# linkedin/spark-tfrecord

Hardware: NVIDIA H100
Metric: TFRecord decode GB/s (1 KB Example, 64 mixed features) at 1/2/4/8 H100 (higher is better)
Workload: dtype u8

## Files before the change

### spark-tfrecord_b200/_native.py

```python
from __future__ import annotations

import ctypes as C
import os
from typing import List, Optional

import numpy as np

from . import _cabi as A
from ._cabi import HostColumn, column_from_ctypes, make_fields, tfr_batch_info, tfr_column, tfr_field
from .sqltypes import StructType

_DIR = os.path.dirname(os.path.abspath(__file__))
LIB_PATH = os.environ.get("TFR_LIB") or os.path.join(_DIR, "libtfrgpu.so")
_LIB = None

EXPORTS = [
    "tfr_abi_version", "tfr_status_string", "tfr_last_error", "tfr_schema_create", "tfr_schema_destroy",
    "tfr_schema_num_fields", "tfr_decoder_create", "tfr_decoder_destroy", "tfr_decoder_staging", "tfr_decoder_staging_slot",
    "tfr_decoder_num_staging_slots", "tfr_decode", "tfr_decode_submit",
    "tfr_decoder_stream", "tfr_decoder_set_profiling", "tfr_decoder_get_profile", "tfr_decoder_get_stats", "tfr_batch_wait", "tfr_batch_status", "tfr_batch_consumed", "tfr_batch_num_columns", "tfr_batch_columns",
    "tfr_batch_to_host_async", "tfr_batch_to_host", "tfr_batch_export_arrow_host", "tfr_batch_export_arrow_device", "tfr_batch_release",
    "tfr_encoder_create", "tfr_encoder_destroy", "tfr_encode", "tfr_encoder_result_host", "tfr_encoder_stream",
    "tfr_infer_create", "tfr_infer_update", "tfr_infer_update_block", "tfr_infer_result", "tfr_infer_name", "tfr_infer_destroy",
]
# ... 232 lines not shown
        h = C.c_void_p()
        _check(lib().tfr_decoder_create(self.schema.h, device, flags, C.byref(h)))
        self.h = h

    def staging(self, nbytes: int) -> np.ndarray:
        p = C.c_void_p()
        cap = C.c_size_t()
        _check(lib().tfr_decoder_staging(self.h, nbytes, C.byref(p), C.byref(cap)))
        return np.ctypeslib.as_array(C.cast(p, C.POINTER(C.c_uint8)), shape=(cap.value,))

    def staging_slot(self, slot: int, nbytes: int) -> np.ndarray:
        p = C.c_void_p()
        cap = C.c_size_t()
        _check(lib().tfr_decoder_staging_slot(self.h, slot, nbytes, C.byref(p), C.byref(cap)))
        return np.ctypeslib.as_array(C.cast(p, C.POINTER(C.c_uint8)), shape=(cap.value,))

    @staticmethod
    def num_staging_slots() -> int:
        return lib().tfr_decoder_num_staging_slots()

    def stats(self) -> dict:
        v = (C.c_int64 * 8)()
        _check(lib().tfr_decoder_get_stats(self.h, v, 8))
        names = ["batches", "speculative_submits", "speculative_redone", "count_mode_batches", "general_path_batches", "shapes_learned", "transcode_reruns"]
        return {k: v[i] for i, k in enumerate(names)}

    def stream(self) -> int:
        p = C.c_void_p()
        _check(lib().tfr_decoder_stream(self.h, C.byref(p)))
        return p.value or 0

    def set_profiling(self, enable: bool):
        _check(lib().tfr_decoder_set_profiling(self.h, 1 if enable else 0))

    def get_profile(self):
        ms = (C.c_double * 8)()
        nl = C.c_int64()
        n1 = C.c_int64()
        _check(lib().tfr_decoder_get_profile(self.h, ms, C.byref(nl), C.byref(n1)))
        names = ["frame_index", "pass1", "scan", "pass2", "pack_validity", "h2d", "d2h"]
        return {"ms": {k: ms[i] for i, k in enumerate(names)}, "launches": nl.value, "pass1_launches": n1.value}

    def decode(self, data, is_final: bool = True, nbytes: Optional[int] = None):
        ptr, n, on_dev, keep = _device_ptr(data)
        if nbytes is not None:
            n = nbytes
        b = C.c_void_p()
# ... 113 lines not shown
```

### spark-tfrecord_b200/csrc/api_decode.inc

```

static inline size_t align_up(size_t v, size_t a) { return (v + a - 1) / a * a; }

struct HostStats {
  FrameResult frame;
  DecodeSummary summary;
  uint32_t overflow;
  uint32_t pad[3];
};

struct K1Bufs {
  DevBuf chunks, chunk_base, first, stage, rec_off;
  uint32_t n_chunks = 0, chunk_bytes = 0;
  void release() { chunks.release(); chunk_base.release(); first.release(); stage.release(); rec_off.release(); }
};

struct PtrTables {
  void** h = nullptr; size_t cap = 0;
  DevBuf dev;
  int32_t ensure(size_t n_ptr) {
    if (cap < n_ptr) {
      if (h) cudaFreeHost(h);
      h = nullptr; cap = 0;
      CUDA_TRY(cudaHostAlloc((void**)&h, n_ptr * sizeof(void*), cudaHostAllocDefault));
      cap = n_ptr;
// ... 50 lines not shown
  Lane lanes[TFR_LANES];
  int next_lane = 0;
  HostStats* h_stats = nullptr;
  int64_t* h_totals = nullptr;
  PinnedPool host_pool;
  DevPool dev_pool;
  std::vector<cudaEvent_t> done_pool;
  bool fast_ok = false;
  int spec_state = 0;
  int relearn_backoff = 0;
  int shape_misses = 0;
  double mean_rec_bytes = 0.0;
  uint32_t last_max_len = 0;
  uint32_t last_max_tile = 0;
  int xc_batches = 0;
  double cap_slack = 0.0625;
  std::vector<int32_t> spec_len;
  bool spec_ragged = false;
  std::vector<double> hist_ratio;
  DevBuf uniform_dev;
  DevBuf no_uniform_dev;
  int32_t* h_uniform = nullptr;
  int64_t stats[8] = {0};
  bool profiling = false;
  struct Span { int stage; cudaEvent_t a, b; };
  std::vector<Span> spans;
  std::vector<cudaEvent_t> ev_pool;
  double prof_ms[TFR_PROFILE_STAGES] = {0};
  int64_t launches = 0, pass1_launches = 0;
  cudaEvent_t ev_get() {
    if (!ev_pool.empty()) { cudaEvent_t e = ev_pool.back(); ev_pool.pop_back(); return e; }
    cudaEvent_t e; cudaEventCreate(&e); return e;
  }
  void span_begin(int stage, cudaStream_t st = nullptr) { if (!profiling) return; Span s{stage, ev_get(), nullptr}; cudaEventRecord(s.a, st ? st : stream); spans.push_back(s); }
  void span_end(int nlaunch, cudaStream_t st = nullptr) { launches += nlaunch; if (!profiling) return; Span& s = spans.back(); s.b = ev_get(); cudaEventRecord(s.b, st ? st : stream); }
  void spans_resolve() {
    const bool trace = !spans.empty() && getenv("TFR_TRACE");
    for (auto& s : spans) {
      if (!s.b) { ev_pool.push_back(s.a); continue; }
      float ms = 0; if (cudaEventElapsedTime(&ms, s.a, s.b) == cudaSuccess) prof_ms[s.stage] += ms;
      if (trace) { float t0 = 0; cudaEventElapsedTime(&t0, spans[0].a, s.a); fprintf(stderr, "tfr_trace stage %d start %.3f end %.3f\n", s.stage, t0, t0 + ms); }
      ev_pool.push_back(s.a); ev_pool.push_back(s.b);
    }
    spans.clear();
  }
};

struct tfr_batch {
  tfr_decoder* dec = nullptr;
  std::atomic<int> refs{1};
  tfr_batch_info info{};
  std::vector<tfr_column> cols;
  std::vector<tfr_column> host_cols;
  void* dev_fixed = nullptr; size_t dev_fixed_bytes = 0;
  void* dev_var = nullptr; size_t dev_var_bytes = 0;
  unsigned long long* d_null_counts = nullptr;
  std::vector<unsigned long long> h_null_counts_tmp;
  void* host_copy = nullptr; size_t host_copy_bytes = 0;
  bool host_copy_enqueued = false;
  cudaEvent_t d2h_done = nullptr;
  bool null_counts_ready = false;
  cudaEvent_t done = nullptr;
  bool pending = false;
  Lane* lane = nullptr;
  const void* src = nullptr; size_t src_bytes = 0; int src_on_device = 0, is_final = 0;
  bool xc_tried = false;
  OutLayout lay;
  std::vector<size_t> lvl_off;
  std::vector<int32_t> uni_len;
};

static void give_event(tfr_decoder* d, cudaEvent_t e) { if (e) d->done_pool.push_back(e); }
static int32_t take_event(tfr_decoder* d, cudaEvent_t* e) {
  if (!d->done_pool.empty()) { *e = d->done_pool.back(); d->done_pool.pop_back(); return TFR_OK; }
  CUDA_TRY(cudaEventCreateWithFlags(e, cudaEventDisableTiming));
  return TFR_OK;
}

extern "C" int32_t tfr_decoder_create(const tfr_schema* schema, int32_t device, uint32_t flags, tfr_decoder** out) {
  if (!schema || !out) return fail(TFR_E_INVALID_ARG, "null argument");
  DeviceCtx* ctx = nullptr;
  int32_t rc = get_ctx(device, &ctx);
  if (rc) return rc;
  CUDA_TRY(cudaSetDevice(device));
  auto* d = new tfr_decoder;
  d->schema = *schema; d->device = device; d->flags = flags; d->ctx = ctx;
  CUDA_TRY(cudaStreamCreateWithFlags(&d->stream, cudaStreamNonBlocking));
  {
    int lo = 0, hi = 0;
    CUDA_TRY(cudaDeviceGetStreamPriorityRange(&lo, &hi));
    CUDA_TRY(cudaStreamCreateWithPriority(&d->st_k1, cudaStreamNonBlocking, getenv("TFR_NO_K1_PRIORITY") ? lo : hi));
  }
  CUDA_TRY(cudaStreamCreateWithFlags(&d->st_h2d, cudaStreamNonBlocking));
  CUDA_TRY(cudaStreamCreateWithFlags(&d->st_d2h, cudaStreamNonBlocking));
  CUDA_TRY(cudaStreamCreateWithFlags(&d->st_aux, cudaStreamNonBlocking));
  rc = d->dsch.upload(d->schema);
  if (!rc) rc = d->dsch.build_tile_consts(d->schema, ctx->d_tabs);
  if (rc) { delete d; return rc; }
  TRY(d->small.ensure(4096 + (size_t)d->schema.n_cnt * 16));
  {
    bool ok = d->schema.fields.size() <= 128 && !getenv("TFR_DISABLE_FAST");
    for (const DevField& f : d->schema.fields) if (f.depth > 1 && d->schema.record_type == TFR_RT_EXAMPLE) ok = false;
    d->fast_ok = ok;
    if (getenv("TFR_DISABLE_SPECULATION")) d->spec_state = -1;
    const size_t nv = std::max(1, d->schema.n_var);
    d->spec_len.assign(nv, -1);
    d->hist_ratio.assign(std::max(1, d->schema.n_cnt), 0.0);
    CUDA_TRY(cudaHostAlloc((void**)&d->h_uniform, nv * 4, cudaHostAllocDefault));
    TRY(d->uniform_dev.ensure(nv * 4));
    TRY(d->no_uniform_dev.ensure(nv * 4));
    CUDA_TRY(cudaMemset(d->no_uniform_dev.p, 0xff, nv * 4));
  }
  CUDA_TRY(cudaHostAlloc((void**)&d->h_stats, sizeof(HostStats), cudaHostAllocDefault));
  size_t nt = (size_t)d->schema.n_cnt * 2 + d->schema.fields.size() + 8;
  CUDA_TRY(cudaHostAlloc((void**)&d->h_totals, nt * sizeof(int64_t), cudaHostAllocDefault));
  for (Lane& L : d->lanes) {
    L.h_res_bytes = sizeof(LaneResult) + 8 * std::max<size_t>(1, d->schema.fields.size()) + 8 * std::max<size_t>(1, (size_t)d->schema.n_cnt);
    TRY(L.res.ensure(L.h_res_bytes));
    CUDA_TRY(cudaHostAlloc((void**)&L.h_res, L.h_res_bytes, cudaHostAllocDefault));
    CUDA_TRY(cudaEventCreateWithFlags(&L.ev_in, cudaEventDisableTiming));
    CUDA_TRY(cudaEventCreateWithFlags(&L.ev_k1, cudaEventDisableTiming));
    CUDA_TRY(cudaEventCreateWithFlags(&L.ev_tile, cudaEventDisableTiming));
    CUDA_TRY(cudaEventCreateWithFlags(&L.ev_frame, cudaEventDisableTiming));
    CUDA_TRY(cudaHostAlloc((void**)&L.h_frame, sizeof(FrameResult), cudaHostAllocDefault));
  }
  *out = d;
  return TFR_OK;
}
static void decoder_unref(tfr_decoder* d);
extern "C" void tfr_decoder_destroy(tfr_decoder* d) { if (d) decoder_unref(d); }
static void decoder_unref(tfr_decoder* d) {
  if (d->refs.fetch_sub(1) != 1) return;
  int prev = -1; cudaGetDevice(&prev);
  cudaSetDevice(d->device);
  for (cudaStream_t s : {d->st_h2d, d->st_k1, d->stream, d->st_d2h, d->st_aux}) cudaStreamSynchronize(s);
  for (DevBuf* b : {&d->in, &d->status, &d->valid8, &d->cnt, &d->src, &d->cflag, &d->tsum, &d->scan_scratch, &d->small, &d->uniform_dev, &d->no_uniform_dev})
    b->release();
  d->k1.release(); d->pt.release();
  for (Lane& L : d->lanes) {
    L.in.release(); L.k1.release(); L.res.release(); L.pt.release(); L.lb.release();
    if (L.h_res) cudaFreeHost(L.h_res);
    if (L.staging) cudaFreeHost(L.staging);
    if (L.ev_in) cudaEventDestroy(L.ev_in);
    if (L.ev_k1) cudaEventDestroy(L.ev_k1);
    if (L.ev_tile) cudaEventDestroy(L.ev_tile);
    if (L.ev_frame) cudaEventDestroy(L.ev_frame);
    if (L.h_frame) cudaFreeHost(L.h_frame);
    if (L.orphan_done) cudaEventDestroy(L.orphan_done);
  }
  d->dsch.free_all();
  cudaFreeHost(d->h_stats); cudaFreeHost(d->h_totals);
  if (d->h_uniform) cudaFreeHost(d->h_uniform);
  d->host_pool.release_all();
  d->dev_pool.release_all();
  for (cudaEvent_t e : d->done_pool) cudaEventDestroy(e);
  d->spans_resolve();
  for (cudaEvent_t e : d->ev_pool) cudaEventDestroy(e);
  for (cudaStream_t s : {d->st_h2d, d->st_k1, d->stream, d->st_d2h, d->st_aux}) cudaStreamDestroy(s);
  delete d;
// ... 303 lines not shown
        A.canon_lean = 1;
        const unsigned long long wgroups = (unsigned long long)((n_eff + 31) / 32) * S.n_var;
        const uint32_t gl = (uint32_t)std::min<unsigned long long>((wgroups + 7) / 8, (unsigned long long)d->ctx->sm_count * 48);
        decode_pass2_canon_kernel<<<std::max<uint32_t>(gl, 1), 256, 0, st>>>(A);
        ++nl2;
      }
      decode_pass2_kernel<<<g2, warps * 32, 0, st>>>(A);
      d->span_end(nl2);
    }
  }
  if (pack && n_eff > 0 && nf > 0) {
    uint32_t nbytes_bm = (n_eff + 7) / 8;
    dim3 g((nbytes_bm + 255) / 256, nf);
    g.x = std::min<uint32_t>(g.x, 4096);
    d->span_begin(4);
    pack_validity_kernel<<<g, 256, 0, st>>>((const uint8_t*)d->valid8.p, n, n_eff, nf, L.nb_stride, C.fx + L.bitmaps_off, b->d_null_counts);
    d->span_end(1);
  }
  build_views(b, S, n_eff, totals, lvl_off);
  return TFR_OK;
}

struct TileGeom { uint32_t tile_cap; uint32_t slot; bool small; size_t smem; uint32_t pf_dist; };
static TileGeom tile_geom_for(const tfr_decoder* d, uint32_t max_len, bool fill, uint32_t rg = 0, uint32_t max_tile = 0) {
  const uint32_t nf = (uint32_t)d->schema.fields.size(), nb = (uint32_t)d->schema.names.size();
  static const size_t l1_keep = getenv("TFR_L1_KEEP_KB") ? (size_t)atoi(getenv("TFR_L1_KEEP_KB")) << 10 : (size_t)16 << 10;
  const size_t sm_bytes = d->ctx->smem_per_sm;
  size_t stride = align_up((size_t)max_len + 16 + 15 + 32, 16);
  if (((stride >> 4) & 1) == 0) stride += 16;
  stride = std::min<size_t>(stride, 1u << 20);
  const size_t cap_fixed = stride * TILE_ROWS;
  TileGeom g;
  auto tiles_per_sm = [&](size_t cap, bool small) { return std::min<size_t>(sm_bytes / (tile_smem_bytes(nf, nb, (uint32_t)cap, rg) + 1024), small ? 8 : TILE_MIN_CTAS); };
  auto is_small = [&](size_t cap) { return (tile_smem_bytes(nf, nb, (uint32_t)cap, rg) + 1024) * 8 <= sm_bytes && d->schema.record_type != TFR_RT_SEQUENCE_EXAMPLE && !getenv("TFR_NO_SMALL_TILES"); };
  size_t cap = cap_fixed;
  g.slot = (uint32_t)stride;
  if (max_tile && !getenv("TFR_NO_PACKED_SIZING")) {
    const size_t cap_packed = std::min<size_t>(cap_fixed, align_up((size_t)max_tile + max_tile / 16 + 2048, 512));
    if (tiles_per_sm(cap_packed, is_small(cap_packed)) > tiles_per_sm(cap_fixed, is_small(cap_fixed))) { cap = cap_packed; g.slot = 0; }
  }
  g.tile_cap = (uint32_t)cap;
  const size_t need = tile_smem_bytes(nf, nb, g.tile_cap, rg) + 1024;
  g.small = is_small(cap);
  const size_t k_max = g.small ? 8 : TILE_MIN_CTAS;
  if (fill && !getenv("TFR_NO_FILL")) {
    const size_t k = std::min<size_t>(sm_bytes / std::max<size_t>(need, 1), k_max);
// ... 192 lines not shown
          for (int v = 0; v < S.n_var; ++v) {
            const DevField& fd = S.fields[S.var_field[v]];
            utot[fd.cnt_slot] = (int64_t)d->spec_len[v] * n;
            if (utot[fd.cnt_slot] > 0x7fffffffLL) return fail(TFR_E_BATCH_TOO_LARGE, "Arrow int32 offsets overflow; decode smaller blocks");
            b->lay.val_off[v] = var_bytes;
            var_bytes += align_up((size_t)utot[fd.cnt_slot] * fd.width + 8, 256);
          }
          if (var_bytes) { b->dev_var = d->dev_pool.acquire(var_bytes); if (!b->dev_var) return fail(TFR_E_OOM, "device allocation failed (batch outputs)"); }
          b->dev_var_bytes = var_bytes;
          for (int v = 0; v < S.n_var; ++v) {
            C.t_vals[v] = (uint8_t*)b->dev_var + b->lay.val_off[v];
            C.t_offs[v * 3 + 0] = C.fx + b->lay.off0_off[v]; C.t_offs[v * 3 + 1] = nullptr; C.t_offs[v * 3 + 2] = nullptr;
          }
          CUDA_TRY(cudaMemcpyAsync(C.dt_offs, C.t_offs, ((size_t)S.n_var * 4) * sizeof(void*), cudaMemcpyHostToDevice, st));
        }
        CUDA_TRY(cudaMemsetAsync(dflags_ptr(d), 0, 4, st));
        TileArgs TA{};
        TA.data = C.d_data; TA.nbytes = (uint32_t)nbytes; TA.misalign = (uint32_t)(reinterpret_cast<uintptr_t>(C.d_data) & 15u); TA.rec_off = (const uint32_t*)d->k1.rec_off.p; TA.n = n; TA.tile_cap = tile_cap; TA.slot = geom.slot; TA.tile_max = nullptr;
        TA.n_dev = nullptr; TA.pf_dist = geom.pf_dist;
        TA.verify = C.verify; TA.names_bytes = names_bytes; TA.sch = d->dsch.view; TA.consts = d->dsch.d_tile_consts; TA.const_bytes = d->dsch.tile_consts_bytes;
        TA.bitmaps = C.fx + b->lay.bitmaps_off; TA.nb_stride = b->lay.nb_stride; TA.null_counts = b->d_null_counts;
        TA.fix_values = A.fix_values; TA.cnt = A.cnt; TA.src = A.src; TA.cflag = A.cflag;
        TA.uniform_len = (const int32_t*)(uniform ? d->uniform_dev.p : d->no_uniform_dev.p); TA.var_values = (void* const*)C.dt_vals; TA.flags = dflags_ptr(d);
        d->span_begin(1);
        TRY(launch_tile(d, TA, n, geom, st));
        d->span_end(1); d->pass1_launches++;
        uint32_t tflags = 0;
        if (uniform) {
          if (S.n_var) {
            d->span_begin(2);
            uniform_offsets_kernel<<<dim3(std::min<uint32_t>((n + 256) / 256, 512), S.n_var), 256, 0, st>>>((int32_t* const*)C.dt_offs, 3, (const int32_t*)d->uniform_dev.p, (uint32_t)S.n_var, n, nullptr);
            d->span_end(1);
          }
          CUDA_TRY(cudaMemcpyAsync(&d->h_stats->overflow, dovf_ptr(d), 8, cudaMemcpyDeviceToHost, st));
          CUDA_TRY(cudaStreamSynchronize(st));
          CUDA_TRY(cudaGetLastError());
          tflags = (&d->h_stats->overflow)[1];
          if (!(tflags & TF_FALLBACK)) {
            for (int a = 0; a < S.n_cnt; ++a) totals[a] = utot[a];
            TRY(finish_var_and_views(C, A, n, totals, false, false));
            done = true;
          } else {
            if (tflags & TF_SHAPE) {
              d->spec_state = 0;
              if (++d->shape_misses >= 2) d->relearn_backoff = 8;
            }
            if (b->dev_var) { d->dev_pool.give_back(b->dev_var, d->stream); b->dev_var = nullptr; b->dev_var_bytes = 0; }
            if (tflags & TF_SHAPE) {
              CUDA_TRY(cudaMemsetAsync(b->d_null_counts, 0, sizeof(unsigned long long) * std::max<uint32_t>(nf, 1), st));
              CUDA_TRY(cudaMemsetAsync(dflags_ptr(d), 0, 4, st));
              TA.uniform_len = (const int32_t*)d->no_uniform_dev.p;
              d->span_begin(1);
              TRY(launch_tile(d, TA, n, geom, st));
              d->span_end(1); d->pass1_launches++;
            }
          }
        }
        if (!done && (!uniform || (tflags & TF_SHAPE))) {
          TRY(scans_and_sync(C, A, false));
          tflags = (&d->h_stats->overflow)[1];
          if (!(tflags & TF_FALLBACK)) {
            if (d->h_stats->overflow)
              for (int a = 0; a < S.n_cnt; ++a) if (totals[a] < 0 || totals[a] > 0x7fffffffLL) return fail(TFR_E_BATCH_TOO_LARGE, "Arrow int32 offsets overflow; decode smaller blocks");
            A.flist_warp = S.record_type == TFR_RT_SEQUENCE_EXAMPLE && !getenv("TFR_DISABLE_FLIST_WARP");
            TRY(finish_var_and_views(C, A, n, totals, true, false));
            done = true;
            d->stats[3]++;
            if (d->relearn_backoff > 0) --d->relearn_backoff;
            else if (d->spec_state == 0) {
              bool ok = true, ragged = false;
              for (int v = 0; v < S.n_var && ok; ++v) {
                const DevField& fd = S.fields[S.var_field[v]];
                const int64_t c0 = totals[S.n_cnt + fd.cnt_slot];
                if (fd.n_levels == 1 && c0 > 0 && totals[fd.cnt_slot] == c0 * (int64_t)n) d->spec_len[v] = (int32_t)c0;
                else if (getenv("TFR_DISABLE_RAGGED")) ok = false;
                else if (fd.depth <= 1) { d->spec_len[v] = TILE_RAGGED; ragged = true; }
                else if (S.record_type == TFR_RT_SEQUENCE_EXAMPLE && S.n_var <= 4 && fd.elem_type != TFR_T_STRING && fd.elem_type != TFR_T_BINARY) {
                  d->spec_len[v] = TILE_RAGGED; ragged = true;
                } else ok = false;
              }
              if (ragged && ((size_t)tile_ragged_bytes((uint32_t)S.n_var, (uint32_t)S.n_cnt) > 24576 || S.n_cnt > 128)) ok = false;
              if (ok) {
                d->spec_state = 1; d->spec_ragged = ragged; d->stats[5]++;
                memcpy(d->h_uniform, d->spec_len.data(), (size_t)S.n_var * 4);
                CUDA_TRY(cudaMemcpyAsync(d->uniform_dev.p, d->h_uniform, (size_t)S.n_var * 4, cudaMemcpyHostToDevice, st));
                CUDA_TRY(cudaStreamSynchronize(st));
              }
            }
            for (int a = 0; a < S.n_cnt; ++a) d->hist_ratio[a] = used ? (double)totals[a] / (double)used : 0.0;
          }
        }
        if (done) { n_eff = n; sum.n_eff = n; if (uniform && !(tflags & TF_FALLBACK)) d->shape_misses = 0; }
      }
      if (!done && !k1_verified) {
        batch_drop_outputs(b);
        allow_fast = false;
        again = true;
      } else if (!done) {
        CUDA_TRY(cudaMemsetAsync(b->d_null_counts, 0, sizeof(unsigned long long) * std::max<uint32_t>(nf, 1), st));
        TRY(ensure_rec_off(C));
        fill_decode_args(C, A);
        const uint32_t warps = 8;
        size_t smem1 = CRC_SMEM_WORDS * 4 + (size_t)warps * ((nf + 3) & ~3u);
        uint32_t g1 = std::min<uint32_t>((n + warps - 1) / warps, (uint32_t)d->ctx->sm_count * 16);
        d->span_begin(1);
        decode_pass1_kernel<<<g1, warps * 32, smem1, st>>>(A);
        d->span_end(1); d->pass1_launches++;
        TRY(scans_and_sync(C, A, true));
        sum = d->h_stats->summary;
        n_eff = sum.n_eff;
        if (sum.first_err_row != 0xffffffffu) used = sum.consumed;
        if (d->h_stats->overflow)
          for (int a = 0; a < S.n_cnt; ++a) if (totals[a] < 0 || totals[a] > 0x7fffffffLL) return fail(TFR_E_BATCH_TOO_LARGE, "Arrow int32 offsets overflow; decode smaller blocks");
        TRY(finish_var_and_views(C, A, n_eff, totals, true));
        d->stats[4]++;
// ... 134 lines not shown
    if (fixed_ready) CUDA_TRY(cudaStreamWaitEvent(sb, fixed_ready, 0));
    d->span_begin(2, sb);
    uniform_offsets_kernel<<<dim3(std::min<uint32_t>((cap + 256) / 256, 512), S.n_var), 256, 0, sb>>>((int32_t* const*)C.dt_offs, 3, (const int32_t*)d->uniform_dev.p, (uint32_t)S.n_var, cap,
                                                                                                  &d_res->frame.n_records);
    d->span_end(1, sb);
  }
  CUDA_TRY(cudaEventRecord(L.ev_k1, sb));
  CUDA_TRY(cudaStreamWaitEvent(d->st_aux, L.ev_k1, 0));
  CUDA_TRY(cudaMemcpyAsync(L.h_frame, &d_res->frame, sizeof(FrameResult), cudaMemcpyDeviceToHost, d->st_aux));
  CUDA_TRY(cudaEventRecord(L.ev_frame, d->st_aux));
  const uint32_t rg = (ragged ? tile_ragged_bytes((uint32_t)S.n_var, (uint32_t)S.n_cnt) : 0u) + (S.record_type == TFR_RT_SEQUENCE_EXAMPLE ? tile_seq_bytes((uint32_t)S.n_var, ragged) : 0u);
  const bool bytes_rows = S.record_type == TFR_RT_BYTE_ARRAY;
  const TileGeom geom = bytes_rows ? bytes_geom_for(d, d->last_max_len, true) : tile_geom_for(d, d->last_max_len, true, rg, d->last_max_tile);
  TileArgs TA{};
  TA.ragged = ragged ? 1u : 0u; TA.n_cnt = (uint32_t)S.n_cnt; TA.ticket = d_ticket; TA.lb_flag = d_lbflag; TA.lb_agg = d_lbagg; TA.lb_pre = d_lbpre;
  TA.cap = d_cap; TA.totals = (unsigned long long*)((uint8_t*)L.res.p + sizeof(LaneResult) + 8 * std::max<size_t>(1, nf));
  TA.offs = (int32_t* const*)C.dt_offs; TA.var_field = d->dsch.d_var_field;
  TA.data = d_data; TA.nbytes = (uint32_t)nbytes; TA.misalign = (uint32_t)(reinterpret_cast<uintptr_t>(d_data) & 15u); TA.rec_off = (const uint32_t*)L.k1.rec_off.p; TA.n = cap; TA.n_dev = &d_res->frame.n_records;
  TA.tile_cap = geom.tile_cap; TA.slot = geom.slot; TA.tile_max = &d_res->max_tile; TA.pf_dist = geom.pf_dist;
  TA.verify = verify; TA.names_bytes = names_bytes; TA.sch = d->dsch.view; TA.consts = d->dsch.d_tile_consts; TA.const_bytes = d->dsch.tile_consts_bytes;
  TA.bitmaps = fx + b->lay.bitmaps_off; TA.nb_stride = b->lay.nb_stride; TA.null_counts = (unsigned long long*)((uint8_t*)L.res.p + sizeof(LaneResult));
  TA.fix_values = (void* const*)C.dt_fix; TA.cnt = nullptr; TA.src = nullptr; TA.cflag = nullptr;
  TA.uniform_len = (const int32_t*)d->uniform_dev.p; TA.var_values = (void* const*)C.dt_vals; TA.flags = &d_res->flags;
  CUDA_TRY(cudaStreamWaitEvent(sa, L.ev_k1, 0));
  d->span_begin(1);
  if (bytes_rows) { TA.tile_max = nullptr; TA.const_bytes = bytes_const_bytes(); TRY(launch_bytes(d, TA, cap, geom, sa)); }
  else TRY(launch_tile(d, TA, cap, geom, sa));
  d->span_end(1); d->pass1_launches++;
  CUDA_TRY(cudaEventRecord(L.ev_tile, sa));
  CUDA_TRY(cudaStreamWaitEvent(d->st_d2h, L.ev_tile, 0));
  CUDA_TRY(cudaMemcpyAsync(L.h_res, L.res.p, L.h_res_bytes, cudaMemcpyDeviceToHost, d->st_d2h));
  if (!b->done) TRY(take_event(d, &b->done));
  CUDA_TRY(cudaEventRecord(b->done, d->st_d2h));
  CUDA_TRY(cudaGetLastError());
  if (d->xc_batches > 0 && ragged) --d->xc_batches;
  b->pending = true;
  L.pending = b;
  d->stats[1]++;
  return TFR_OK;
}

static int32_t resolve(tfr_batch* b) {
  if (!b->pending) return TFR_OK;
  NvtxRange nvtx("tfr_batch_resolve");
  tfr_decoder* d = b->dec;
  Lane& L = *b->lane;
// ... 10 lines not shown
    b->info.n_records = n; b->info.n_rows = n; b->info.frame_repairs = (int32_t)fr.repairs;
    b->info.consumed_bytes = (int64_t)frame_used(fr, b->src_bytes, b->is_final != 0);
    if (frame_err) { b->info.error_code = frame_err; b->info.error_row = n; b->info.error_field = -1; }
    std::vector<int64_t> totals(std::max(1, S.n_cnt), 0);
    const unsigned long long* dev_tot = (const unsigned long long*)((const uint8_t*)L.h_res + sizeof(LaneResult) + 8 * std::max<size_t>(1, S.fields.size()));
    for (int v = 0; v < S.n_var; ++v) {
      const DevField& fd = S.fields[S.var_field[v]];
      if (b->uni_len[v] >= 0) totals[fd.cnt_slot] = (int64_t)b->uni_len[v] * n;
      else for (int l = 0; l < fd.n_levels; ++l) totals[fd.cnt_slot + l] = (int64_t)dev_tot[fd.cnt_slot + l];
    }
    if (b->lvl_off.size() < (size_t)S.n_var * 3) b->lvl_off.assign((size_t)S.n_var * 3, 0);
    build_views(b, S, n, totals.data(), b->lvl_off);
    if (!frame_err && b->info.consumed_bytes > 0)
      for (int a = 0; a < S.n_cnt; ++a) d->hist_ratio[a] = (double)totals[a] / (double)b->info.consumed_bytes;
    const unsigned long long* nc = (const unsigned long long*)(L.h_res + 1);
    for (size_t f = 0; f < b->cols.size(); ++f) b->cols[f].null_count = n ? (int64_t)nc[f] : 0;
    b->null_counts_ready = true;
    if (n > 64 && !frame_err) {
      const double est = (double)b->src_bytes / d->mean_rec_bytes, err = est > 0 ? fabs((double)n - est) / est : 1.0;
      d->cap_slack = std::min(0.0625, std::max(0.01, 8.0 * err));
      d->mean_rec_bytes = (double)fr.stop_pos / n; d->last_max_len = fr.max_len; d->last_max_tile = r.max_tile;
    }
    d->shape_misses = 0;
    d->stats[0]++;
    return TFR_OK;
  }
  if ((r.flags & TF_XCODE) && !(r.flags & (TF_SHAPE | TF_OVERFLOW)) && !b->xc_tried && fr.n_records <= b->lay.n_alloc && d->spec_state == 1) {
    b->xc_tried = true;
    d->xc_batches = 64;
    const uint32_t cap = b->lay.n_alloc;
    batch_drop_outputs(b);
    b->host_copy_enqueued = false; b->host_cols.clear();
    if (b->d2h_done) CUDA_TRY(cudaEventSynchronize(b->d2h_done));
    if (b->host_copy) { d->host_pool.give_back(b->host_copy); b->host_copy = nullptr; }
    d->stats[6]++;
    TRY(submit_async(d, L, b, b->src, b->src_bytes, 1, b->is_final, cap));
    return resolve(b);
  }
  d->stats[2]++;
  if (fr.n_records > b->lay.n_alloc) d->cap_slack = 0.0625;
  const bool unlearned = (r.flags & TF_SHAPE) && d->spec_state == 1;
  if (r.flags & TF_SHAPE) {
    d->spec_state = 0;
    if (++d->shape_misses >= 2) d->relearn_backoff = 8;
  }
  batch_drop_outputs(b);
  b->host_copy_enqueued = false; b->host_cols.clear();
  if (b->d2h_done) CUDA_TRY(cudaEventSynchronize(b->d2h_done));
  if (b->host_copy) { d->host_pool.give_back(b->host_copy); b->host_copy = nullptr; }
  TRY(decode_sync(d, b, b->src, b->src_bytes, 1, b->is_final, true));
  if (unlearned && b->info.error_code && d->spec_state == 0) { d->spec_state = 1; if (d->shape_misses > 0) --d->shape_misses; d->relearn_backoff = 0; }
  return TFR_OK;
}

static int32_t lane_make_free(tfr_decoder* d, Lane& L) {
  if (L.pending) TRY(resolve(L.pending));
  if (L.orphan_done) {
    CUDA_TRY(cudaEventSynchronize(L.orphan_done));
    give_event(d, L.orphan_done); L.orphan_done = nullptr;
    const LaneResult r = *L.h_res;
    if (r.flags & TF_FALLBACK) d->stats[2]++;
    if (r.flags & TF_SHAPE) { d->spec_state = 0; if (++d->shape_misses >= 2) d->relearn_backoff = 8; }
    else if (!(r.flags & TF_FALLBACK) && r.frame.n_records > 64) { d->mean_rec_bytes = (double)r.frame.stop_pos / r.frame.n_records; d->last_max_len = r.frame.max_len; d->last_max_tile = r.max_tile; }
  }
  return TFR_OK;
}

extern "C" int32_t tfr_decode_submit(tfr_decoder* d, const void* data, size_t nbytes, int32_t data_on_device, int32_t is_final, tfr_batch** out) {
  if (!d || !out || (nbytes && !data)) return fail(TFR_E_INVALID_ARG, "null argument");
  if (nbytes >= (1ull << 31)) return fail(TFR_E_BATCH_TOO_LARGE, "tfr_decode: a batch must be smaller than 2 GiB; split the file at record boundaries");
  NvtxRange nvtx("tfr_decode_submit");
  std::lock_guard<std::recursive_mutex> lk(d->mu);
  CUDA_TRY(cudaSetDevice(d->device));
  auto* b = new tfr_batch;
  b->dec = d;
  d->refs.fetch_add(1);
  std::unique_ptr<tfr_batch, void (*)(tfr_batch*)> guard(b, [](tfr_batch* x) { tfr_batch_release(x); });
  uint32_t cap = 0;
  if (can_speculate(d, data, nbytes, data_on_device, &cap)) {
    int li = -1;
    if (!data_on_device)
      for (int k = 0; k < TFR_LANES; ++k) if (d->lanes[k].staging && data == d->lanes[k].staging) li = k;
    if (li < 0) { li = d->next_lane; d->next_lane = (d->next_lane + 1) % TFR_LANES; }
    Lane& L = d->lanes[li];
    TRY(lane_make_free(d, L));
// ... 159 lines not shown
```

### spark-tfrecord_b200/csrc/tile.cuh

```cuda
#pragma once
#include "common.cuh"
#include "decode.cuh"

#define TILE_ROWS 32
#ifndef TILE_PARSE_WARPS
#define TILE_PARSE_WARPS 12
#endif
#ifndef TILE_CRC_WARPS
#define TILE_CRC_WARPS 3
#endif
#define TILE_THREADS ((TILE_PARSE_WARPS + TILE_CRC_WARPS) * 32)
#ifndef TILE_MIN_CTAS
#define TILE_MIN_CTAS 3
#endif
#define TILE_TPL_WORDS 5

struct FieldTemplate {
  uint32_t words[TILE_TPL_WORDS];
  uint32_t mask[TILE_TPL_WORDS];
  uint16_t n_words;
  uint16_t klen;
  uint32_t kind;
};

// ... 13 lines not shown
  DevSchema sch;
  const uint8_t* consts;
  uint32_t const_bytes;
  uint8_t* bitmaps;
  uint32_t nb_stride;
  unsigned long long* null_counts;
  void* const* fix_values;
  uint32_t* cnt;
  uint32_t* src;
  uint8_t* cflag;
  const int32_t* uniform_len;
  uint32_t ragged;
  uint32_t n_cnt;
  uint32_t* ticket;
  uint32_t* lb_flag;
  uint32_t* lb_agg;
  unsigned long long* lb_pre;
  const unsigned long long* cap;
  unsigned long long* totals;
  int32_t* const* offs;
  const int32_t* var_field;
  void* const* var_values;
  uint32_t* flags;
};

enum { TF_FALLBACK = 1u, TF_SHAPE = 2u, TF_OVERFLOW = 4u, TF_XCODE = 8u };
#define TILE_RAGGED (-2)

__device__ __forceinline__ uint32_t smem_u32(const void* p) { return (uint32_t)__cvta_generic_to_shared(p); }
__device__ __forceinline__ void mbar_init(uint64_t* bar, uint32_t count) {
  asm volatile("mbarrier.init.shared::cta.b64 [%0], %1;" ::"r"(smem_u32(bar)), "r"(count));
}
__device__ __forceinline__ void mbar_expect_tx(uint64_t* bar, uint32_t bytes) {
  asm volatile("mbarrier.arrive.expect_tx.shared::cta.b64 _, [%0], %1;" ::"r"(smem_u32(bar)), "r"(bytes) : "memory");
}
__device__ __forceinline__ void bulk_g2s(void* dst, const void* src, uint32_t bytes, uint64_t* bar) {
  asm volatile("cp.async.bulk.shared::cluster.global.mbarrier::complete_tx::bytes [%0], [%1], %2, [%3];" ::"r"(smem_u32(dst)),
               "l"(src), "r"(bytes), "r"(smem_u32(bar))
               : "memory");
}
__device__ __forceinline__ void mbar_wait(uint64_t* bar, uint32_t phase) {
  uint32_t ok;
  do {
    asm volatile(
        "{\n"
        ".reg .pred p;\n"
        "mbarrier.try_wait.parity.shared::cta.b64 p, [%1], %2;\n"
        "selp.u32 %0, 1, 0, p;\n"
        "}\n"
// ... 232 lines not shown
      }
      const uint32_t k0 = K * cw / CW, k1 = K * (cw + 1) / CW;
      c = crc_chunks(s8, T, b0 + 16 * k0, k1 - k0, c);
      if (c) atomicXor(&scrc[lane], K - k1 ? gf2_mulmod(xp16[K - k1], c) : c);
    }
    asm volatile("bar.sync 2, %0;" ::"r"(CW * 32) : "memory");
    if (cw == 0 && on) {
      uint32_t c = scrc[lane];
      for (uint32_t o = b0 + 16 * K; o < end; ++o) c = crc_byte(s8, c, T.u8(o));
      if (crc_mask(~c) != t_u32(T, end)) atomicOr(A.flags, TF_FALLBACK);
    }
    if (cw == CW - 1 && A.pf_dist) {
      const uint32_t row2 = (tile + A.pf_dist) * TILE_ROWS + lane;
      if (row2 < n_rows) {
        const uint32_t o2 = A.rec_off[row2] + mis, e2 = min(A.rec_off[row2 + 1] + mis, lim & ~15u);
        const uint32_t a2 = (o2 + 15u) & ~15u;
        if (e2 > a2 + 16u) asm volatile("cp.async.bulk.prefetch.L2.global [%0], %1;" ::"l"(base + a2), "r"((e2 - a2) & ~15u) : "memory");
      }
    }
    return;
  }

  bool bad = false;
  uint32_t skip = wid;
  uint32_t shape_bad = 0;
  unsigned long long seen_lo = 0, seen_hi = 0;
  if (active) {
    uint32_t p = pay, L = 0;
    uint32_t cend = end, fl_start = end, fl_end = end;
    if (len < 2 || T.u8(p) != 0x0A) bad = true;
    else {
      ++p;
      if (!t_len(T, p, end, L) || end - p < L) bad = true;
      else if (!SEQ) { if (p + L != end) bad = true; }
      else {
        cend = p + L;
        uint32_t q = cend, L2 = 0;
        if (q >= end || T.u8(q) != 0x12) bad = true;
        else { ++q; if (!t_len(T, q, end, L2) || q + L2 != end) bad = true; else { fl_start = q; fl_end = end; } }
      }
    }
    uint32_t next_f = wid;
    while (!bad && p < cend) {
      for (bool wide = true; wide;) {
        wide = false;
        while (skip && p < cend) {
          const int32_t b1 = T.i8(p + 1);
          if (b1 < 0) { wide = true; break; }
          p += 2u + (uint32_t)b1;
          --skip;
        }
        if (wide) {
          uint32_t q = p + 1, el;
          if (!t_len(T, q, cend, el)) { bad = true; break; }
          p = q + el;
          --skip;
        }
      }
      if (bad || p >= cend) break;
      skip = PW - 1;
      uint32_t eend, kind, llen;
      int f = -1;
      bool located = false;
      if (next_f < nf && stpl[next_f].n_words) {
        const FieldTemplate& tp = stpl[next_f];
        const uint32_t klen = tp.klen;
        const uint32_t ab = p & ~3u, sh = (p & 3u) * 8;
        uint32_t aw[TILE_TPL_WORDS + 1];
#pragma unroll
        for (int w = 0; w <= TILE_TPL_WORDS; ++w) aw[w] = T.w32(ab + 4 * w);
        uint32_t diff = 0, u0 = 0;
#pragma unroll
        for (int w = 0; w < TILE_TPL_WORDS; ++w) {
          const uint32_t u = __funnelshift_r(aw[w], aw[w + 1], sh);
          if (w == 0) u0 = u;
          diff |= (u ^ tp.words[w]) & tp.mask[w];
        }
        const uint32_t elen = (u0 >> 8) & 0xff, vl = T.u8(p + 5 + klen), ll = T.u8(p + 7 + klen);
        if (diff == 0 && elen < 0x80 && elen == klen + 4 + vl && vl == ll + 2 && p + 2 + elen <= cend) {
          f = (int)next_f; eend = p + 2 + elen; located = true;
          kind = tp.kind; llen = ll;
          p += klen + 8;
        }
      }
      if (!located) {
        uint32_t elen, klen, vlen;
        if (T.u8(p) != 0x0A) { bad = true; break; }
        ++p;
        if (!t_len(T, p, cend, elen) || cend - p < elen) { bad = true; break; }
        eend = p + elen;
        if (p >= eend || T.u8(p) != 0x0A) { bad = true; break; }
        ++p;
        if (!t_len(T, p, eend, klen) || eend - p < klen) { bad = true; break; }
        const uint32_t key = p;
        p += klen;
        if (p >= eend || T.u8(p) != 0x12) { bad = true; break; }
        ++p;
        if (!t_len(T, p, eend, vlen) || p + vlen != eend) { bad = true; break; }
        uint32_t hi = 0;
        for (uint32_t i = 0; i < klen; ++i) hi |= T.u8(key + i);
        if (hi >= 0x80 && !utf8_valid(T.b + key, klen)) { bad = true; break; }
        uint32_t h = name_hash(T.b + key, klen);
        uint32_t slot = h & (uint32_t)A.sch.ht_mask;
        for (;;) {
          int cand = A.sch.ht[slot];
          if (cand < 0) break;
          if (sfields[cand].hash == h && sfields[cand].name_len == klen) {
            const uint8_t* nm = snames + sfields[cand].name_off;
            uint32_t diff = 0;
// ... 159 lines not shown
                  } else for (uint32_t i = 0; i < n; ++i) dst[i] = t_u32(T, pk + 4 * i);
                } else {
                  double* dst = reinterpret_cast<double*>(A.var_values[fd->var_slot]) + (size_t)row * n;
                  for (uint32_t i = 0; i < n; ++i) dst[i] = (double)__uint_as_float(t_u32(T, pk + 4 * i));
                }
              } else {
                uint32_t q = pk;
                for (uint32_t e = 0; e < n; ++e) {
                  uint64_t v = 0; uint32_t sh = 0;
                  for (;;) { uint32_t b = T.u8(q++); v |= (uint64_t)(b & 0x7f) << sh; sh += 7; if (b < 0x80) break; }
                  if (fd->elem_type == TFR_T_INT64) reinterpret_cast<int64_t*>(A.var_values[fd->var_slot])[(size_t)row * n + e] = (int64_t)v;
                  else reinterpret_cast<int32_t*>(A.var_values[fd->var_slot])[(size_t)row * n + e] = (int32_t)(uint32_t)v;
                }
              }
            } else {
              A.cnt[(size_t)fd->cnt_slot * A.n + row] = n;
              A.src[(size_t)fd->var_slot * A.n + row] = pk + g0;
              A.cflag[(size_t)fd->var_slot * A.n + row] = CF_CANON;
            }
          }
        }
      }
      p = eend;
    }
    if (p != cend) bad = true;
    p = fl_start;
    while (SEQ && !bad && p < fl_end) {
      const bool owner = skip == 0;
      skip = owner ? PW - 1 : skip - 1;
      uint32_t elen, klen, vlen;
      if (T.u8(p) != 0x0A) { bad = true; break; }
      ++p;
      const uint32_t entry_pos = p;
      if (!t_len(T, p, fl_end, elen) || fl_end - p < elen) { bad = true; break; }
      const uint32_t eend = p + elen;
      if (p >= eend || T.u8(p) != 0x0A) { bad = true; break; }
      ++p;
      if (!t_len(T, p, eend, klen) || eend - p < klen) { bad = true; break; }
      const uint32_t key = p;
      p += klen;
      if (p >= eend || T.u8(p) != 0x12) { bad = true; break; }
      ++p;
      if (!t_len(T, p, eend, vlen) || p + vlen != eend) { bad = true; break; }
      if (owner) {
        uint32_t hi = 0;
        for (uint32_t i = 0; i < klen; ++i) hi |= T.u8(key + i);
// ... 94 lines not shown
        if (tot_bytes) atomicAdd(&sq_cnt[(fd->var_slot * 32 + lane) * 2 + 1], tot_bytes);
        if (owner) {
          if (RG && A.uniform_len[fd->var_slot] == TILE_RAGGED) {
            if (steps > TILE_SQ_STEPS) { bad = true; break; }
            rg_src[fd->var_slot * 32 + lane] = steps_start;
            rg_cnt[fd->cnt_slot * 32 + lane] = steps;
          } else {
            A.cnt[(size_t)fd->cnt_slot * A.n + row] = steps;
            A.src[(size_t)fd->var_slot * A.n + row] = entry_pos + g0;
            A.cflag[(size_t)fd->var_slot * A.n + row] = CF_FLIST;
          }
        }
      }
      p = eend;
    }
    if (!bad && p != fl_end) bad = true;
  }
  {
    const uint32_t w4[4] = {(uint32_t)seen_lo, (uint32_t)(seen_lo >> 32), (uint32_t)seen_hi, (uint32_t)(seen_hi >> 32)};
#pragma unroll
    for (int k = 0; k < 4; ++k)
      if (w4[k] && (atomicOr(&sseen[lane * 4 + k], w4[k]) & w4[k])) bad = true;
    if (bad) atomicOr(&sseen[160], 1u << lane);
  }
  asm volatile("bar.sync 1, %0;" ::"r"(PW * 32) : "memory");
  if (RG) {
    if (XC && sseen[161]) {
      for (uint32_t v = wid; v < (uint32_t)A.sch.n_var; v += PW) {
        const DevField& fd = sfields[A.var_field[v]];
        if (A.uniform_len[v] != TILE_RAGGED || fd.elem_type != TFR_T_STRING || !active || rg_cnt[fd.cnt_slot * 32 + lane] == 0u || !(rg_src[v * 32 + lane] >> 31)) continue;
        const uint32_t src = rg_src[v * 32 + lane] & 0x7fffffffu;
        if (fd.depth == 0) {
          uint32_t k = 1;
          while (k < 5 && (T.u8(src - 1 - k) & 0x80u)) ++k;
          uint32_t q = src - k, raw = 0;
          t_len(T, q, src, raw);
          rg_cnt[fd.cnt_slot * 32 + lane] = t_xcode_cell(T.b + src, raw, nullptr);
        } else if (fd.depth == 1) {
          const uint32_t cnt = rg_cnt[fd.cnt_slot * 32 + lane];
          uint32_t q = src, tot = 0;
          for (uint32_t i = 0; i < cnt; ++i) { uint32_t bl = 0; ++q; t_len(T, q, q + 5, bl); tot += t_xcode_cell(T.b + q, bl, nullptr); q += bl; }
          rg_cnt[(fd.cnt_slot + 1) * 32 + lane] = tot;
        }
      }
      asm volatile("bar.sync 1, %0;" ::"r"(PW * 32) : "memory");
    }
// ... 237 lines not shown
```

Baseline: 904.5.

## Skip non-owned feature entries via precomputed constant entry-length hops

```diff
diff --git a/spark-tfrecord_b200/_native.py b/spark-tfrecord_b200/_native.py
--- a/spark-tfrecord_b200/_native.py
+++ b/spark-tfrecord_b200/_native.py
@@ -278,7 +278,8 @@
     def stats(self) -> dict:
         v = (C.c_int64 * 8)()
         _check(lib().tfr_decoder_get_stats(self.h, v, 8))
-        names = ["batches", "speculative_submits", "speculative_redone", "count_mode_batches", "general_path_batches", "shapes_learned", "transcode_reruns"]
+        names = ["batches", "speculative_submits", "speculative_redone", "count_mode_batches", "general_path_batches", "shapes_learned", "transcode_reruns",
+                 "constant_hop_submits"]
         return {k: v[i] for i, k in enumerate(names)}
 
     def stream(self) -> int:
diff --git a/spark-tfrecord_b200/csrc/api_decode.inc b/spark-tfrecord_b200/csrc/api_decode.inc
--- a/spark-tfrecord_b200/csrc/api_decode.inc
+++ b/spark-tfrecord_b200/csrc/api_decode.inc
@@ -96,6 +96,9 @@
   DevBuf no_uniform_dev;
   int32_t* h_uniform = nullptr;
   int64_t stats[8] = {0};
+  DevBuf lens_dev;
+  bool lens_set = false;
+  bool layout_ok = true;
   bool profiling = false;
   struct Span { int stage; cudaEvent_t a, b; };
   std::vector<Span> spans;
@@ -142,6 +145,7 @@
   OutLayout lay;
   std::vector<size_t> lvl_off;
   std::vector<int32_t> uni_len;
+  bool hop = false;
 };
 
 static void give_event(tfr_decoder* d, cudaEvent_t e) { if (e) d->done_pool.push_back(e); }
@@ -183,6 +187,7 @@
     CUDA_TRY(cudaHostAlloc((void**)&d->h_uniform, nv * 4, cudaHostAllocDefault));
     TRY(d->uniform_dev.ensure(nv * 4));
     TRY(d->no_uniform_dev.ensure(nv * 4));
+    TRY(d->lens_dev.ensure(2 * std::max<size_t>(1, d->schema.fields.size()) * 4));
     CUDA_TRY(cudaMemset(d->no_uniform_dev.p, 0xff, nv * 4));
   }
   CUDA_TRY(cudaHostAlloc((void**)&d->h_stats, sizeof(HostStats), cudaHostAllocDefault));
@@ -208,7 +213,7 @@
   int prev = -1; cudaGetDevice(&prev);
   cudaSetDevice(d->device);
   for (cudaStream_t s : {d->st_h2d, d->st_k1, d->stream, d->st_d2h, d->st_aux}) cudaStreamSynchronize(s);
-  for (DevBuf* b : {&d->in, &d->status, &d->valid8, &d->cnt, &d->src, &d->cflag, &d->tsum, &d->scan_scratch, &d->small, &d->uniform_dev, &d->no_uniform_dev})
+  for (DevBuf* b : {&d->in, &d->status, &d->valid8, &d->cnt, &d->src, &d->cflag, &d->tsum, &d->scan_scratch, &d->small, &d->uniform_dev, &d->no_uniform_dev, &d->lens_dev})
     b->release();
   d->k1.release(); d->pt.release();
   for (Lane& L : d->lanes) {
@@ -558,6 +563,38 @@
 }
 
 struct TileGeom { uint32_t tile_cap; uint32_t slot; bool small; size_t smem; uint32_t pf_dist; };
+static uint32_t* lens_ptr(tfr_decoder* d, bool small) { return d->lens_set ? (uint32_t*)d->lens_dev.p + (small ? d->schema.fields.size() : 0) : nullptr; }
+static int32_t set_entry_lens(tfr_decoder* d, cudaStream_t st) {
+  const tfr_schema& S = d->schema;
+  const size_t nf = S.fields.size();
+  d->lens_set = false;
+  if (S.record_type != TFR_RT_EXAMPLE || d->spec_ragged || nf == 0) return TFR_OK;
+  std::vector<uint32_t> e(nf, 0), tab(2 * nf, 0);
+  for (size_t f = 0; f < nf; ++f) {
+    const DevField& fd = S.fields[f];
+    const uint32_t klen = fd.name_len;
+    if (fd.kind == K_NONE || fd.depth > 1 || klen + 8 > TILE_TPL_WORDS * 4) continue;
+    const int32_t u = fd.var_slot >= 0 ? d->spec_len[fd.var_slot] : -1;
+    if (fd.var_slot >= 0 && u < 0) continue;
+    int64_t list = -1;
+    if (fd.kind == K_FLOAT) { const int64_t n = fd.depth == 0 ? 1 : u; if (4 * n < 128) list = 2 + 4 * n; }
+    else if (fd.kind == K_BYTES && fd.depth == 0 && u < 128) list = 2 + u;
+    if (list >= 0 && klen + 6 + list < 128) e[f] = (uint32_t)(klen + 8 + list);
+  }
+  for (int t = 0; t < 2; ++t) {
+    const size_t W = t ? 4 : 12;
+    for (size_t f = 0; f < nf; ++f) {
+      uint32_t c = 0;
+      if (f + W - 1 < nf) for (size_t j = f + 1; j < f + W; ++j) { if (!e[j]) { c = 0; break; } c += e[j]; }
+      tab[t * nf + f] = e[f] | (c << 16);
+    }
+  }
+  CUDA_TRY(cudaMemcpyAsync(d->lens_dev.p, tab.data(), tab.size() * 4, cudaMemcpyHostToDevice, st));
+  CUDA_TRY(cudaStreamSynchronize(st));
+  d->lens_set = true;
+  return TFR_OK;
+}
+
 static TileGeom tile_geom_for(const tfr_decoder* d, uint32_t max_len, bool fill, uint32_t rg = 0, uint32_t max_tile = 0) {
   const uint32_t nf = (uint32_t)d->schema.fields.size(), nb = (uint32_t)d->schema.names.size();
   static const size_t l1_keep = getenv("TFR_L1_KEEP_KB") ? (size_t)atoi(getenv("TFR_L1_KEEP_KB")) << 10 : (size_t)16 << 10;
@@ -796,6 +833,7 @@
         TA.bitmaps = C.fx + b->lay.bitmaps_off; TA.nb_stride = b->lay.nb_stride; TA.null_counts = b->d_null_counts;
         TA.fix_values = A.fix_values; TA.cnt = A.cnt; TA.src = A.src; TA.cflag = A.cflag;
         TA.uniform_len = (const int32_t*)(uniform ? d->uniform_dev.p : d->no_uniform_dev.p); TA.var_values = (void* const*)C.dt_vals; TA.flags = dflags_ptr(d);
+        TA.lens = uniform ? lens_ptr(d, geom.small) : nullptr; TA.hop_on = 0;
         d->span_begin(1);
         TRY(launch_tile(d, TA, n, geom, st));
         d->span_end(1); d->pass1_launches++;
@@ -823,7 +861,7 @@
             if (tflags & TF_SHAPE) {
               CUDA_TRY(cudaMemsetAsync(b->d_null_counts, 0, sizeof(unsigned long long) * std::max<uint32_t>(nf, 1), st));
               CUDA_TRY(cudaMemsetAsync(dflags_ptr(d), 0, 4, st));
-              TA.uniform_len = (const int32_t*)d->no_uniform_dev.p;
+              TA.uniform_len = (const int32_t*)d->no_uniform_dev.p; TA.lens = nullptr;
               d->span_begin(1);
               TRY(launch_tile(d, TA, n, geom, st));
               d->span_end(1); d->pass1_launches++;
@@ -858,13 +896,14 @@
                 d->spec_state = 1; d->spec_ragged = ragged; d->stats[5]++;
                 memcpy(d->h_uniform, d->spec_len.data(), (size_t)S.n_var * 4);
                 CUDA_TRY(cudaMemcpyAsync(d->uniform_dev.p, d->h_uniform, (size_t)S.n_var * 4, cudaMemcpyHostToDevice, st));
+                TRY(set_entry_lens(d, st));
                 CUDA_TRY(cudaStreamSynchronize(st));
               }
             }
             for (int a = 0; a < S.n_cnt; ++a) d->hist_ratio[a] = used ? (double)totals[a] / (double)used : 0.0;
           }
         }
-        if (done) { n_eff = n; sum.n_eff = n; if (uniform && !(tflags & TF_FALLBACK)) d->shape_misses = 0; }
+        if (done) { n_eff = n; sum.n_eff = n; if (uniform && !(tflags & TF_FALLBACK)) d->shape_misses = 0; d->layout_ok = !(tflags & TF_LAYOUT); }
       }
       if (!done && !k1_verified) {
         batch_drop_outputs(b);
@@ -1045,6 +1084,14 @@
   TA.bitmaps = fx + b->lay.bitmaps_off; TA.nb_stride = b->lay.nb_stride; TA.null_counts = (unsigned long long*)((uint8_t*)L.res.p + sizeof(LaneResult));
   TA.fix_values = (void* const*)C.dt_fix; TA.cnt = nullptr; TA.src = nullptr; TA.cflag = nullptr;
   TA.uniform_len = (const int32_t*)d->uniform_dev.p; TA.var_values = (void* const*)C.dt_vals; TA.flags = &d_res->flags;
+  if (!bytes_rows && !ragged && S.record_type == TFR_RT_EXAMPLE && d->lens_set) {
+    TA.lens = lens_ptr(d, geom.small);
+#ifndef TFR_NO_LENS_HOP
+    TA.hop_on = d->layout_ok ? 1u : 0u;
+#endif
+  }
+  b->hop = TA.hop_on != 0;
+  if (b->hop) d->stats[7]++;
   CUDA_TRY(cudaStreamWaitEvent(sa, L.ev_k1, 0));
   d->span_begin(1);
   if (bytes_rows) { TA.tile_max = nullptr; TA.const_bytes = bytes_const_bytes(); TRY(launch_bytes(d, TA, cap, geom, sa)); }
@@ -1101,6 +1148,7 @@
       d->mean_rec_bytes = (double)fr.stop_pos / n; d->last_max_len = fr.max_len; d->last_max_tile = r.max_tile;
     }
     d->shape_misses = 0;
+    d->layout_ok = !(r.flags & TF_LAYOUT);
     d->stats[0]++;
     return TFR_OK;
   }
@@ -1118,8 +1166,10 @@
   }
   d->stats[2]++;
   if (fr.n_records > b->lay.n_alloc) d->cap_slack = 0.0625;
-  const bool unlearned = (r.flags & TF_SHAPE) && d->spec_state == 1;
-  if (r.flags & TF_SHAPE) {
+  if (r.flags & TF_LAYOUT) d->layout_ok = false;
+  const bool shape_miss = (r.flags & TF_SHAPE) && !(b->hop && (r.flags & TF_LAYOUT));
+  const bool unlearned = shape_miss && d->spec_state == 1;
+  if (shape_miss) {
     d->spec_state = 0;
     if (++d->shape_misses >= 2) d->relearn_backoff = 8;
   }
@@ -1139,7 +1189,8 @@
     give_event(d, L.orphan_done); L.orphan_done = nullptr;
     const LaneResult r = *L.h_res;
     if (r.flags & TF_FALLBACK) d->stats[2]++;
-    if (r.flags & TF_SHAPE) { d->spec_state = 0; if (++d->shape_misses >= 2) d->relearn_backoff = 8; }
+    if (r.flags & TF_LAYOUT) d->layout_ok = false;
+    if ((r.flags & TF_SHAPE) && !(r.flags & TF_LAYOUT)) { d->spec_state = 0; if (++d->shape_misses >= 2) d->relearn_backoff = 8; }
     else if (!(r.flags & TF_FALLBACK) && r.frame.n_records > 64) { d->mean_rec_bytes = (double)r.frame.stop_pos / r.frame.n_records; d->last_max_len = r.frame.max_len; d->last_max_tile = r.max_tile; }
   }
   return TFR_OK;
diff --git a/spark-tfrecord_b200/csrc/tile.cuh b/spark-tfrecord_b200/csrc/tile.cuh
--- a/spark-tfrecord_b200/csrc/tile.cuh
+++ b/spark-tfrecord_b200/csrc/tile.cuh
@@ -59,9 +59,11 @@
   const int32_t* var_field;
   void* const* var_values;
   uint32_t* flags;
+  const uint32_t* lens;
+  uint32_t hop_on;
 };
 
-enum { TF_FALLBACK = 1u, TF_SHAPE = 2u, TF_OVERFLOW = 4u, TF_XCODE = 8u };
+enum { TF_FALLBACK = 1u, TF_SHAPE = 2u, TF_OVERFLOW = 4u, TF_XCODE = 8u, TF_LAYOUT = 16u };
 #define TILE_RAGGED (-2)
 
 __device__ __forceinline__ uint32_t smem_u32(const void* p) { return (uint32_t)__cvta_generic_to_shared(p); }
@@ -340,6 +342,7 @@
   }
 
   bool bad = false;
+  bool layout_miss = false;
   uint32_t skip = wid;
   uint32_t shape_bad = 0;
   unsigned long long seen_lo = 0, seen_hi = 0;
@@ -380,6 +383,7 @@
       uint32_t eend, kind, llen;
       int f = -1;
       bool located = false;
+      uint32_t hop_c = 0;
       if (next_f < nf && stpl[next_f].n_words) {
         const FieldTemplate& tp = stpl[next_f];
         const uint32_t klen = tp.klen;
@@ -398,11 +402,18 @@
         if (diff == 0 && elen < 0x80 && elen == klen + 4 + vl && vl == ll + 2 && p + 2 + elen <= cend) {
           f = (int)next_f; eend = p + 2 + elen; located = true;
           kind = tp.kind; llen = ll;
+          if (A.lens) {
+            const uint32_t lx = __ldg(&A.lens[next_f]), el = lx & 0xffffu;
+            if (el && el != elen + 2) { layout_miss = true; if (A.hop_on) { bad = true; break; } }
+            hop_c = lx >> 16;
+          }
           p += klen + 8;
         }
       }
       if (!located) {
         uint32_t elen, klen, vlen;
+        layout_miss = true;
+        if (A.hop_on) { bad = true; break; }
         if (T.u8(p) != 0x0A) { bad = true; break; }
         ++p;
         if (!t_len(T, p, cend, elen) || cend - p < elen) { bad = true; break; }
@@ -608,6 +619,7 @@
         }
       }
       p = eend;
+      if (A.hop_on && hop_c && p + hop_c <= cend) { p += hop_c; skip = 0; }
     }
     if (p != cend) bad = true;
     p = fl_start;
@@ -748,6 +760,7 @@
     for (int k = 0; k < 4; ++k)
       if (w4[k] && (atomicOr(&sseen[lane * 4 + k], w4[k]) & w4[k])) bad = true;
     if (bad) atomicOr(&sseen[160], 1u << lane);
+    if (__any_sync(FULLMASK, layout_miss) && lane == 0) atomicOr(A.flags, TF_LAYOUT);
   }
   asm volatile("bar.sync 1, %0;" ::"r"(PW * 32) : "memory");
   if (RG) {
```

Result: no change. 902.3 (median of 6 runs) (-0.2%).
